# JorgeDFR/nmpc_nav_control

Hardware: AMD Instinct MI355X
Metric: SQP-RTI iterations/sec (whole node), diff N=40 batch=4096; u0 max-abs err (higher is better)
Workload: dtype fp32+fp64; 1 GPU; diff2amr N=40 batch=4096 per GPU; config=metric, N=40, batch_per_gpu=4096, global_batch=4096, parallelism=instance-sharded x1, ranks=1, launcher=single process, closed_loop_warmup_ticks=240, rccl_gather=False, full=False, ipm_rules=product

## Files before the change

### nmpc_nav_control_amd/csrc/sqp_rti_team.hip

```cpp
#include "nmpc_kernels.hpp"
#include "team_common.hpp"
#include "sqp_steps.hpp"
#include "path_march.hpp"

namespace nmpc {

#ifdef NMPC_STAMPS
constexpr int kStampIts = 64;
__device__ unsigned long long g_stamps[256][2 + 4 * kStampIts];
#define STAMP(slot)                                                                                              \
    do {                                                                                                         \
        if (r == 0 && (team & 3) == 0 && (team >> 2) < 256) g_stamps[team >> 2][(slot)] = __builtin_amdgcn_s_memtime(); \
    } while (0)
__device__ unsigned long long g_stamps_p1[256][8];
__device__ unsigned long long g_stamps_pa[256];
__device__ unsigned long long g_stamps_c1[256][kStampIts];
#define STAMPC1()                                                                                                \
    do {                                                                                                         \
        if (it < kStampIts && r == 0 && (team & 3) == 0 && (team >> 2) < 256)                                   \
            g_stamps_c1[team >> 2][it] = __builtin_amdgcn_s_memtime();                                           \
    } while (0)
#define STAMPF(slot)                                                                                             \
    do {                                                                                                         \
        if (it == 2 && k == 20 && r == 0 && (team & 3) == 0 && (team >> 2) < 256)                                 \
            g_stamps_p1[team >> 2][(slot)] = __builtin_amdgcn_s_memtime();                                        \
    } while (0)
#else
#define STAMP(slot) ((void)0)
#define STAMPF(slot) ((void)0)
#define STAMPC1() ((void)0)
#endif

template <class M>
size_t team_scratch_floats(int N, int stride)
{
    return (size_t)stride * (N + 1) * 16 * (TeamRec<M>::RSS + 1) + (size_t)256 * 4 * 16 * (TeamRec<M>::RSS + 1) + 64;
}

namespace {
#ifndef LIGHT_D
#define LIGHT_D 4
#endif
#ifndef LIGHT_DC
#define LIGHT_DC LIGHT_D
#endif
#ifndef P1_D
#define P1_D 2
#endif
#ifdef NMPC_STAMPS
constexpr int kStampItsC = kStampIts;
#else
constexpr int kStampItsC = 0;
#endif

__device__ float g_zero4[4];
__device__ __attribute__((aligned(16))) float g_rec_sentinel[8] = {kFar, kFar, 0.0f, 0.0f, -kFar, kFar, 0.0f, 0.0f};

constexpr int kModeRunPath = 2;
template <class M, bool MS, bool SD, int MODE, bool SP, bool RP, bool MT>
__global__ __launch_bounds__(256, 1) void k_sqp_rti_team(KParams P, KArgs a)
{
    constexpr int mode = MODE == kModeRunPath ? kModeRun : MODE;
    using R = TeamRec<M, SD>;
    constexpr int NX = M::NX, NU = M::NU, NV = R::NV, NGV = R::NGV, RS = R::RS, RSS = R::RSS;
    constexpr bool QM = rec_quad_major<NV>();
    constexpr int KS = 16 * RSS;
    const int gt = blockIdx.x * blockDim.x + threadIdx.x;
    const int team = a.split ? (int)blockIdx.x : (gt >> 4);
    const int row = a.split ? (int)(threadIdx.x >> 4) : 0;
    const int r = gt & 15;
    if (team >= a.B) return;
    if (a.n_active && team >= *a.n_active) return;
    const int N = P.N;
    const size_t S = (size_t)a.stride;
    const size_t Bn = (size_t)a.B;
    const int inst = a.order ? a.order[team] : team;
    const LaneCtx<M> lc = lane_ctx<M, RP>(P, a, inst, r);
    const bool lv = lc.lv, is_u = lc.is_u, is_x = lc.is_x, has_b = lc.has_b;
    const int xi = lc.xi, cx = lc.cx;
    const float sc = P.dt, w_lane = lc.w_lane, h_stage = lc.h_stage, lo_b = lc.lo_b, hi_b = lc.hi_b;
    StageBox sbx{};
    if constexpr (RP) sbx = stage_box_ctx<M, MT>(a, inst, lc, r);
    ModelVals mvals{};
    if constexpr (MT) mvals = robot_vals<M>(P, a, inst);
    const ModelPar mp = MT ? model_par(P, mvals) : model_par(P);
    float* const tbase = a.scratch + (size_t)inst * (N + 1) * KS + (lv ? r : 0) * rec_lane<RSS, QM>();
    float* const tbase_own = a.scratch + (size_t)inst * (N + 1) * KS + r * rec_lane<RSS, QM>();
    float* const tdummy = a.scratch + (size_t)inst * (N + 1) * KS + (size_t)N * KS + 15 * rec_lane<RSS, QM>();
    constexpr bool SPL = R::SPLIT_OK && SP;
    float* const pc0 = a.scratch + (size_t)inst * (N + 1) * KS + (lv ? r : 0) * R::CW;
    float* const pb0 = has_b ? a.scratch + (size_t)inst * (N + 1) * KS + (size_t)(N + 1) * R::CS +
                                   (is_u ? r : NU + (cx >= 0 ? cx : 0)) * R::CW
                             : g_rec_sentinel;
    const int kb = has_b ? R::BS : 0;
    float* const dzbase = a.scratch + (size_t)a.sstride * (N + 1) * KS + (size_t)inst * (N + 1) * 16 + r;
    const bool warm = P.warm && a.warm && a.warm[inst] == a.warm_tag && !(a.reset && a.reset[inst]);

#define XB(k, j) a.xbar[((size_t)(k) * NX + (j)) * S + inst]
#define UBAR(k, j) a.ubar[((size_t)(k) * NU + (j)) * S + inst]

    STAMP(0);
    if (a.reset && a.reset[inst]) {
        for (int k = r; k <= N; k += 16)
            for (int j = 0; j < NX; j++) XB(k, j) = 0.0f;
        for (int k = r; k < N; k += 16)
            for (int j = 0; j < NU; j++) UBAR(k, j) = 0.0f;
        __threadfence_block();
    }

    extern __shared__ double s_path[];
    constexpr bool path = MODE == kModeRunPath;
    const bool traj_lds = path || (a.split && mode == kModeRun);
    const int nslot = a.split ? 1 : 16;
    const int tslot = a.split ? 0 : (int)(threadIdx.x >> 4);
    float* const my_traj = reinterpret_cast<float*>(s_path + nslot * (N + 1)) + (size_t)tslot * (N + 1) * 3;
    float* const s_stg = reinterpret_cast<float*>(s_path) + (traj_lds ? (size_t)nslot * (N + 1) * 5 : 0);
    if (path && row == 0) {
        double* const my_u = s_path + (size_t)tslot * (N + 1);
        const nmpc_path_segment* S = a.segs + (size_t)inst * a.seg_stride;
        const int n = a.nseg[inst];
        if (r == 0) {
            const int cnt = path_march(S, n, a.nearest_u[inst], a.period, N + 1, [&](int j, double su) { my_u[j] = su; });
            for (int j = cnt; j <= N; j++) my_u[j] = (double)n;
        }
        const double* const fr = a.origin();
        const double ox = fr ? fr[inst] : 0.0, oy = fr ? fr[(size_t)a.sstride + inst] : 0.0;
        for (int j = r; j <= N; j += 16) {
            double px, py, pt;
            path_pose(S, n, my_u[j], a.holo, &px, &py, &pt);
            const float fx = (float)(px - ox), fy = (float)(py - oy);
            my_traj[j * 3 + 0] = fx;
            my_traj[j * 3 + 1] = fy;
            my_traj[j * 3 + 2] = (float)pt;
            if (a.traj_out) {
                a.traj_out[((size_t)j * 3 + 0) * Bn + inst] = fx;
                a.traj_out[((size_t)j * 3 + 1) * Bn + inst] = fy;
                a.traj_out[((size_t)j * 3 + 2) * Bn + inst] = (float)pt;
            }
        }
    }

    float x0[NX];
    const X0Lane xl = load_x0<M, RP>(P, a, mode, inst, lc, mp, x0);
    const float pose_th = xl.pose_th, x0_lane = xl.x0_lane;
    float we_lane = xl.we_lane;

    using SL = StageLds<M>;
    if (a.split) {
        const int len_a = (mode == kModeRun) ? ((a.traj_len && !path) ? a.traj_len[inst] : N + 1) : 0;
        struct In {
            float x[NX], u[NU], y, xnext, tq;
            float2 l;
        };
        auto ld = [&](int k, In& v) {
            const int kk = k <= N ? k : N;
#pragma unroll
            for (int j = 0; j < NX; j++) v.x[j] = XB(kk, j);
            const int ku = kk < N ? kk : N - 1;
#pragma unroll
            for (int j = 0; j < NU; j++) v.u[j] = UBAR(ku, j);
            v.xnext = XB(kk < N ? kk + 1 : N, xi);
            v.y = 0.0f;
            v.tq = 0.0f;
            if (mode != kModeRun) {
                const int j = is_u ? NX + r : xi;
                v.y = (lv && j < a.ny_in) ? a.yref[((size_t)kk * a.ny_in + j) * Bn + inst] : 0.0f;
            } else if (!path && r < 3) {
                const int kt = kk < len_a ? kk : (len_a > 0 ? len_a - 1 : 0);
                v.tq = a.traj[((size_t)kt * 3 + r) * Bn + inst];
            }
            v.l = warm ? *reinterpret_cast<const float2*>(SPL ? pb0 + (size_t)kk * kb + 2
                                                              : tbase + (size_t)kk * KS + rec_off<RS, QM>(R::LL))
                       : make_float2(0.0f, 0.0f);
        };
        In cur, nxt;
        ld(row, cur);
        for (int k = row; k <= N; k += 16) {
            ld(k + 16, nxt);
            if (mode == kModeRun && !path && r < 3) my_traj[k * 3 + r] = cur.tq;
            const P0In<M> in = p0_stage_inputs<M>(P, mp, lc, r, k, N, cur.x, cur.u, cur.xnext);
            float* const st = s_stg + SL::at(k, r);
            st[SL::ZBAR] = in.zb;
            st[SL::YREF] = cur.y;
            st[SL::LL] = cur.l.x;
            st[SL::LU] = cur.l.y;
            st[SL::DEFECT] = in.bk;
#pragma unroll
            for (int i = 0; i < NGV; i++) st[SL::gv(i)] = in.g[i];
            cur = nxt;
        }
        __syncthreads();
        if (row != 0) return;
#ifdef NMPC_STAMPS
        if (r == 0 && (team & 3) == 0 && (team >> 2) < 256) g_stamps_pa[team >> 2] = __builtin_amdgcn_s_memtime();
#endif
    }
    const int len = (mode == kModeRun) ? ((a.traj_len && !path) ? a.traj_len[inst] : N + 1) : 0;
    RefUnwrap ref(pose_th);
    float prv_x = 0.0f, prv_y = 0.0f, prv_t = 0.0f;
    auto load_row = [&](int k, float (&xr)[NX], float (&ur)[NU], float (&tr)[3]) {
        const int kk = k <= N ? k : N;
#pragma unroll
        for (int j = 0; j < NX; j++) xr[j] = XB(kk, j);
        const int ku = kk < N ? kk : N - 1;
#pragma unroll
        for (int j = 0; j < NU; j++) ur[j] = UBAR(ku, j);
        if (mode == kModeRun) {
            const int kt = kk < len ? kk : (len > 0 ? len - 1 : 0);
#pragma unroll
            for (int j = 0; j < 3; j++) tr[j] = path ? my_traj[kt * 3 + j] : a.traj[((size_t)kt * 3 + j) * Bn + inst];
        } else {
            tr[0] = tr[1] = tr[2] = 0.0f;
        }
    };
    float xb[NX], ub[NU], tr[3], xb1[NX], ub1[NU], tr1[3];
    load_row(0, xb, ub, tr);
    load_row(1, xb1, ub1, tr1);
    float gcol[NX], grow[NV];
    const_rows<M>(P, mp, lc, r, xb, ub, gcol, grow);
    float dx = is_x ? x0_lane - XB(0, xi) : 0.0f;
    float sum_c0 = 0.0f;
    auto load_l = [&](int k) -> float2 {
        const int kk = k <= N ? k : N;
        const float* const src = warm ? (SPL ? pb0 + (size_t)kk * kb + 2 : tbase + (size_t)kk * KS + rec_off<RS, QM>(R::LL))
                                      : g_zero4;
        return *reinterpret_cast<const float2*>(src);
    };
    auto p0_body = [&](int k, float zbar, float yr_in, const float (&trk)[3], float2 lp, const float (&g)[NX],
                       float bk, float2 box) __attribute__((always_inline)) {
        float yr = yr_in;
        if (mode == kModeRun) {
            ref.step(k < len, trk);
            if (k == N - 1) { prv_x = ref.ref_x; prv_y = ref.ref_y; prv_t = ref.ref_t; }
            float v = 0.0f;
            v = (is_x && xi == 2) ? ref.ref_t : v;
            v = (is_x && xi == 1) ? ref.ref_y : v;
            v = (is_x && xi == 0) ? ref.ref_x : v;
            yr = v;
        }
        float rec[RS];
#pragma unroll
        for (int f = 0; f < RS; f++) rec[f] = 0.0f;
        const bool vu = is_u && k < N, vx = is_x && k >= 1;
        const bool valid = vu || vx;
        float w = sc * w_lane;
        if (k == N) {
            if (mode == kModeRun && P.terminal_hack)
                we_lane = terminal_weight(lc, we_lane, ref.ref_x == prv_x && ref.ref_y == prv_y && ref.ref_t == prv_t);
            w = vx ? we_lane : w;
        }
        rec[R::GR] = valid ? w * (zbar - yr) : 0.0f;
        if constexpr (RP) rec[R::GR] = stage_box_poison(rec[R::GR], box, valid && has_b);
        const float z = vx ? dx : 0.0f;
        rec[R::Z] = z;
        {
            const BoundStart b = bound_start(P, zbar, z, RP ? box.x : lo_b, RP ? box.y : hi_b, warm, lp, valid && has_b);
            rec[R::LB] = b.lb;
            rec[R::UB] = b.ub;
            rec[R::TL] = b.tl;
            rec[R::TU] = b.tu;
            rec[R::LL] = b.ll;
            rec[R::LU] = b.lu;
            sum_c0 += b.c0;
        }
#pragma unroll
        for (int i = 0; i < NGV; i++) rec[R::GV + i] = (k < N && lv) ? g[i] : 0.0f;
        if constexpr (NV > 12) rec_store_range<0, RSS, RS, QM>(tbase_own + (size_t)k * KS, rec);
        else if constexpr (SPL)
            split_store<R, 0, R::GR + 1, RS>(lv ? pc0 + (size_t)k * R::CS : tdummy,
                                             (lv && has_b) ? pb0 + (size_t)k * kb : tdummy + R::CW, rec);
        else rec_store_range<0, RSS, RS, QM>(lv ? tbase + (size_t)k * KS : tdummy, rec);
        dzbase[(size_t)k * 16] = 0.0f;
        if (k < N) {
            const float dzd = is_x ? dx : 0.0f;
            float nxt = dot_v<NX, NU>(0.0f, dzd, grow);
#pragma unroll
            for (int i = 0; i < NGV; i++) {
                const float sr = row_sum16(lv ? g[i] * dzd : 0.0f);
                if (xi == i) nxt = sr;
            }
            dx = is_x ? nxt + bk : 0.0f;
        }
    };
    if (a.split) {
        __builtin_amdgcn_s_waitcnt(0);
        struct Stg {
            float zb, y, ll, lu, b, g[NGV], t[3];
        };
        auto lds_ld = [&](int k, Stg& o) {
            const int kk = k <= N ? k : N;
            const float* const st = s_stg + SL::at(kk, r);
            o.zb = st[SL::ZBAR];
            o.y = st[SL::YREF];
            o.ll = st[SL::LL];
            o.lu = st[SL::LU];
            o.b = st[SL::DEFECT];
#pragma unroll
            for (int i = 0; i < NGV; i++) o.g[i] = st[SL::gv(i)];
#pragma unroll
            for (int j = 0; j < 3; j++) o.t[j] = (mode == kModeRun) ? my_traj[kk * 3 + j] : 0.0f;
        };
        Stg cur, nxt;
        lds_ld(0, cur);
        float2 box = make_float2(lo_b, hi_b), box_n = box;
        if constexpr (RP) box = stage_box<MT>(sbx, 0, N);
        for (int k = 0; k <= N; k++) {
            lds_ld(k + 1, nxt);
            if constexpr (RP) box_n = stage_box<MT>(sbx, k + 1, N);
            float g[NX];
#pragma unroll
            for (int i = 0; i < NX; i++) g[i] = (i < NGV && k < N) ? cur.g[i < NGV ? i : 0] : 0.0f;
            p0_body(k, cur.zb, cur.y, cur.t, make_float2(cur.ll, cur.lu), g, cur.b, box);
            cur = nxt;
            box = box_n;
        }
    } else {
        struct Row {
            float xb[NX], ub[NU], tr[3], yr;
            float2 lp, bx;
        };
        auto load_p0 = [&](int k, Row& o) {
            load_row(k, o.xb, o.ub, o.tr);
            o.lp = load_l(k);
            if constexpr (RP) o.bx = stage_box<MT>(sbx, k, N);
            o.yr = 0.0f;
            if (mode != kModeRun) {
                const int kk = k <= N ? k : N;
                const int j = is_u ? NX + r : xi;
                const bool use = lv && j < a.ny_in;
                const float v = a.yref[((size_t)kk * a.ny_in + (use ? j : 0)) * Bn + inst];
                o.yr = use ? v : 0.0f;
            }
        };
        Row rw[3];
#pragma unroll
        for (int j = 0; j < NX; j++) { rw[0].xb[j] = xb[j]; rw[1].xb[j] = xb1[j]; }
#pragma unroll
        for (int j = 0; j < NU; j++) { rw[0].ub[j] = ub[j]; rw[1].ub[j] = ub1[j]; }
#pragma unroll
        for (int j = 0; j < 3; j++) { rw[0].tr[j] = tr[j]; rw[1].tr[j] = tr1[j]; }
        rw[0].lp = load_l(0);
        rw[1].lp = load_l(1);
        if constexpr (RP) {
            rw[0].bx = stage_box<MT>(sbx, 0, N);
            rw[1].bx = stage_box<MT>(sbx, 1, N);
        }
        rw[0].yr = rw[1].yr = 0.0f;
        if (mode != kModeRun) {
            Row t0, t1;
            load_p0(0, t0);
            load_p0(1, t1);
            rw[0].yr = t0.yr;
            rw[1].yr = t1.yr;
        }
        for (int k0 = 0;; k0 += 3) {
            bool stop = false;
            sfor<0, 3>([&](auto ic) {
                constexpr int i = decltype(ic)::value;
                if (stop) return;
                const int k = k0 + i;
                load_p0(k + 2, rw[(i + 2) % 3]);
                const Row& c = rw[i];
                const Row& n1 = rw[(i + 1) % 3];
                float dxn[NX], g[NX];
#pragma unroll
                for (int q = 0; q < NX; q++) { dxn[q] = 0.0f; g[q] = 0.0f; }
                if (k < N) rk4_column<M>(c.xb, c.ub, P, mp, lv ? r : NU, dxn, g);
                float zbar = 0.0f;
#pragma unroll
                for (int j = 0; j < NU; j++)
                    if (r == j) zbar = c.ub[j];
#pragma unroll
                for (int j = 0; j < NX; j++)
                    if (is_x && xi == j) zbar = c.xb[j];
                float bk = 0.0f;
#pragma unroll
                for (int q = 0; q < NX; q++)
                    if (xi == q) bk = (c.xb[q] - n1.xb[q]) + dxn[q];
                p0_body(k, zbar, c.yr, c.tr, c.lp, g, bk, RP ? c.bx : make_float2(lo_b, hi_b));
                if (k == N) stop = true;
            });
            if (stop) break;
        }
    }
    double onehot[NV];
#pragma unroll
    for (int j = 0; j < NV; j++) onehot[j] = (r == j) ? 1.0 : 0.0;
    double gcol64[NX];
#pragma unroll
    for (int i = 0; i < NX; i++) gcol64[i] = (double)gcol[i];
#ifdef NMPC_MROW
    constexpr bool kMcol = false;
#else
    constexpr bool kMcol = M::kMcolForm;
#endif
    GConst<M> gcs;
    if constexpr (kMcol && !MT) gconst_load<M>(gcs, gcol);

    STAMP(1);
    const float wmax = (RP && a.rparams) ? row_max16(w_lane) : P.wmax;
    const float lam_thr = P.infeas_lam * fmaxf(1.0f, fmaxf(wmax, row_max16(is_x ? we_lane : 0.0f)) * 0.1f);
    const int m = N * NU + N * M::NBX;
    const float inv_m2 = 0.5f / (float)m;
    sum_c0 = row_sum16(lv ? sum_c0 : 0.0f);

    auto p1_load = [&](int kk, float (&v)[RS]) {
        if constexpr (SPL) split_load<R, R::P1L0, R::P1L1, RS>(pc0 + (size_t)kk * R::CS, pb0 + (size_t)kk * kb, v);
        else rec_load_range<R::P1L0, R::P1L1, RS, QM>(tbase + (size_t)kk * KS, v);
        v[R::DZ] = dzbase[(size_t)kk * 16];
    };
    auto sweep = [&](int k0, int k1, int dir, bool ld, auto&& body) {
        const int sd = ld ? dir : 0;
        int kp = k0;
        float ra[RS], rb[RS];
        p1_load(kp, ra);
        for (int k = k0;; k += 2 * dir) {
            const int kp1 = (k == k1) ? kp : kp + sd;
            p1_load(kp1, rb);
            body(k, ra);
            if (k == k1) break;
            const int kp2 = (k + dir == k1) ? kp1 : kp1 + sd;
            p1_load(kp2, ra);
            body(k + dir, rb);
            if (k + dir == k1) break;
            kp = kp2;
        }
    };
    auto sweepd = [&](auto dc, auto f0c, auto fc, int k0, int k1, int dir, bool ld, auto&& body) {
        constexpr int D = decltype(dc)::value;
        constexpr int F0 = decltype(f0c)::value, F = decltype(fc)::value;
        const int sd = ld ? dir : 0;
        float buf[D][RS];
        int kp = k0;
        int kl = k0;
        auto load = [&](int kk, float (&v)[RS]) {
            if constexpr (SPL) split_load<R, F0, F, RS>(pc0 + (size_t)kk * R::CS, pb0 + (size_t)kk * kb, v);
            else rec_load_range<F0, F, RS, QM>(tbase + (size_t)kk * KS, v);
            if constexpr (F == R::P1L1) v[R::DZ] = dzbase[(size_t)kk * 16];
        };
        load(kp, buf[0]);
        sfor<1, D>([&](auto ic) {
            constexpr int i = decltype(ic)::value;
            kp = (kl == k1) ? kp : kp + sd;
            kl = (kl == k1) ? kl : kl + dir;
            load(kp, buf[i]);
        });
        for (int k = k0;; k += D * dir) {
            bool stop = false;
            sfor<0, D>([&](auto ic) {
                constexpr int i = decltype(ic)::value;
                if (stop) return;
                body(k + i * dir, buf[i]);
                if (k + i * dir == k1) {
                    stop = true;
                    return;
                }
                kp = (kl == k1) ? kp : kp + sd;
                kl = (kl == k1) ? kl : kl + dir;
                load(kp, buf[i]);
            });
            if (stop) break;
        }
    };
    int status = 0, it_done = 0;
    bool done = false;
    float exit_res[3] = {0.0f, 0.0f, 0.0f};
    float alpha = 0.0f, sigma_mu = 0.0f, eta = 0.0f, mu_prev = 3.0e38f;
    float tg_rhs = P.sd_hi * sum_c0 * inv_m2;
    for (int it = 0;; it++) {
        double Lrow[NV];
#pragma unroll
        for (int j = 0; j < NV; j++) Lrow[j] = 0.0;
        float pv = 0.0f, piv = 0.0f;
        float res_stat = 0.0f, res_ineq = 0.0f, sum_c = 0.0f, max_c = 0.0f, stat_scale = 1.0f, nanf_ = 0.0f;
        float lam_max = 0.0f;
        bool fail = false;
        const bool act = lv && !done;
        const float a_upd = (it > 0 && !done) ? alpha : 0.0f;
#if P1_D > 2
        sweepd(std::integral_constant<int, P1_D>{}, std::integral_constant<int, R::P1L0>{},
               std::integral_constant<int, R::P1L1>{}, N, 0, -1, act, [&](int k, float (&rc)[RS]) {
#else
        sweep(N, 0, -1, act, [&](int k, float (&rc)[RS]) {
#endif
            STAMPF(0);
            const bool vu = is_u && k < N;
            const bool vx = is_x && k >= 1;
            const bool valid = vu || vx;
            const bool bnd = valid && has_b;
            float z = rc[R::Z];
            float tl = rc[R::TL], tu = rc[R::TU], ll = rc[R::LL], lu = rc[R::LU];
            const float lb = rc[R::LB], ubd = rc[R::UB];
            {
                const float dz = rc[R::DZ];
                const float rl = z - lb - tl, rr = ubd - z - tu;
                const float itl = frcp(tl), itu = frcp(tu);
                float tgl = sigma_mu, tgu = sigma_mu;
                if constexpr (!SD) {
                    const BoundDir da = bound_dir(rc[R::DZA], rl, rr, tl, tu, ll, lu, itl, itu, 0.0f, 0.0f);
                    tgl = sigma_mu - eta * da.dll * da.dtl;
                    tgu = sigma_mu - eta * da.dlu * da.dtu;
                }
                const BoundDir d = bound_dir(dz, rl, rr, tl, tu, ll, lu, itl, itu, tgl, tgu);
                const float ab = bnd ? a_upd : 0.0f, av = valid ? a_upd : 0.0f;
                tl += ab * d.dtl;
                tu += ab * d.dtu;
                ll += ab * d.dll;
                lu += ab * d.dlu;
                z += av * dz;
                rc[R::Z] = z;
                rc[R::TL] = tl;
                rc[R::TU] = tu;
                rc[R::LL] = ll;
                rc[R::LU] = lu;
            }
            const float rl = z - lb - tl, rr = ubd - z - tu;
            const float itl = frcp(tl), itu = frcp(tu);
            res_ineq = fmaxf(res_ineq, fmaxf(fabsf(rl), fabsf(rr)));
            sum_c += ll * tl + lu * tu;
            max_c = fmaxf(max_c, fmaxf(ll * tl, lu * tu));
            lam_max = fmaxf(lam_max, fmaxf(ll, lu));
            const float lamdiff = ll - lu;
            const float sig = ll * itl + lu * itu;
            const float gh = SD ? ll * rl * itl + ll - lu * rr * itu - lu - tg_rhs * itl + tg_rhs * itu
                                : ll * rl * itl + ll - lu * rr * itu - lu;
            STAMPF(1);
            float Gc[NX];
            stage_column<M, R::GV>(rc, gcol, Gc);
            const float cpi = (k < N) ? dot_x<NX, NU>(0.0f, piv, Gc) : 0.0f;
            const float hz = ((k < N) ? h_stage : we_lane) * z;
            const float g = rc[R::GR];
            const float base = hz + g - lamdiff + cpi;
            rc[R::RU] = base;
            res_stat = fmaxf(res_stat, vu ? fabsf(base) : 0.0f);
            stat_scale = fmaxf(stat_scale, vu ? fmaxf(fabsf(cpi), fmaxf(fabsf(g), fabsf(lamdiff))) : 0.0f);
            const float ghat = valid ? (vu ? gh + base : gh) : 0.0f;
            const float pi_new = vx ? base : 0.0f;
            if (ghat != ghat || sig != sig) nanf_ = 1.0f;
            if (k == N) {
                const double d = is_x ? (double)fmaxf(we_lane + sig, 0.0f) : 0.0;
#pragma unroll
                for (int j = 0; j < NV; j++) Lrow[j] = (is_x && j == r) ? d : 0.0;
                pv = is_x ? ghat : 0.0f;
            } else {
                double Gd[NX];
#pragma unroll
                for (int l = 0; l < NX; l++) Gd[l] = (l < NGV) ? (double)Gc[l] : gcol64[l];
                double pg[NX];
#pragma unroll
                for (int i = 0; i < NX; i++) pg[i] = 0.0;
                STAMPF(2);
                pg_block<NX, NU>(pg, Lrow, Gd);
                STAMPF(3);
                const double dg = valid ? (double)h_stage + (double)sig : 1.0;
                double Lr[NV];
#pragma unroll
                for (int j = 0; j < NV; j++) Lr[j] = onehot[j] * dg;
                double pivot;
                bool seq_pivots = true;
                if constexpr (kMcol) {
                    double m11, m10;
                    if constexpr (MT) m_block_team<M>(Lr, pivot, m11, m10, pg, Gd);
                    else m_block<M>(Lr, pivot, m11, m10, pg, Gd, gcs);
                    STAMPF(4);
                    if constexpr (NU == 2 && M::kPivotsUpFront) {
                        chol_input_2<NX>(Lr, pivot, m11, m10, r, fail);
                        seq_pivots = false;
                    } else {
                        (void)m11;
                        (void)m10;
                    }
                } else {
                    mrow_pg_block<NX, NU>(Lr, pivot, pg, Gd);
                    STAMPF(4);
                }
                if (seq_pivots) sfor<0, NU>([&](auto jc) {
                    constexpr int j = decltype(jc)::value;
                    if (!(pivot > 0.0)) fail = true;
                    const double rd = drsq(fmax(pivot, 1e-300));
                    const double lj = (r >= j) ? Lr[j] * rd : 0.0;
                    Lr[j] = lj;
                    chol_update<NX, NU, j>(Lr, lj, pivot);
                });
                STAMPF(5);
                float Lm[NU];
#pragma unroll
                for (int q = 0; q < NU; q++) {
                    Lm[q] = (float)Lr[q];
                    rc[R::LM + q] = Lm[q];
                }
                float y = dot_x<NX, NU>(ghat, pv, Gc);
                float my_lr = 0.0f;
                sfor<0, NU>([&](auto jc) {
                    constexpr int j = decltype(jc)::value;
                    const float lrj = bc<j>(y * frcp(Lm[j]));
                    if (r == j) my_lr = lrj;
                    y -= Lm[j] * lrj;
                });
                rc[R::LR] = my_lr;
                pv = is_x ? y : 0.0f;
#pragma unroll
                for (int j = 0; j < NV; j++) Lrow[j] = Lr[j];
            }
            piv = pi_new;
            STAMPF(6);
            float* const pk = act ? tbase + (size_t)k * KS : tdummy;
            if constexpr (SPL) {
                split_store<R, 0, R::TL, RS>(act ? pc0 + (size_t)k * R::CS : tdummy, tdummy + R::CW, rc);
                split_store<R, R::TL, R::TL + 4, RS>(tdummy, (act && bnd) ? pb0 + (size_t)k * kb : tdummy + R::CW, rc);
            } else if constexpr (MS) {
                rec_store_range<R::TL, R::TL + 4, RS, QM>(bnd ? pk : tdummy, rc);
                if constexpr (R::TL > 0) rec_store_range<0, R::TL, RS, QM>(pk, rc);
                if constexpr (R::TL + 4 < R::P1S1) rec_store_range<R::TL + 4, R::P1S1, RS, QM>(pk, rc);
            } else {
                rec_store_range<0, R::P1S1, RS, QM>(pk, rc);
            }
            STAMPF(7);
        });
        if (it < kStampItsC) STAMP(2 + 4 * it);
        sum_c = row_sum16(lv ? sum_c : 0.0f);
        max_c = row_max16(lv ? max_c : 0.0f);
        lam_max = row_max16(lv ? lam_max : 0.0f);
        res_ineq = row_max16(lv ? res_ineq : 0.0f);
        res_stat = row_max16(lv ? res_stat : 0.0f);
        stat_scale = row_max16(stat_scale);
        nanf_ = row_max16(nanf_);
        const float failf = row_max16(fail ? 1.0f : 0.0f);
        const float mu = sum_c * inv_m2;
        if (!done) {
            exit_res[0] = res_stat;
            exit_res[1] = res_ineq;
            exit_res[2] = mu;
            bool stop = false;
            if (nanf_ > 0.0f || mu != mu) {
                status = 1;
                stop = true;
            } else if (failf > 0.0f) {
                status = (mu <= kBreakdownMuT && res_ineq <= P.tol_ineq * 10.0f) ? 0 : 4;
                stop = true;
            } else if (lam_max > lam_thr && res_ineq > kInfeasRes) {
                status = 4;
                stop = true;
            } else {
                const bool stat_ok = res_stat <= P.tol_stat || res_stat <= kStatRelT * stat_scale;
                const bool cmax_ok = max_c <= kCompMaxRatio * P.tol_comp;
                const bool stalled = mu <= P.tol_comp && mu > 0.5f * mu_prev;
                if (res_ineq <= P.tol_ineq &&
                    ((stat_ok && mu <= P.tol_comp && cmax_ok) || mu <= 1e-2f * P.tol_comp || (stalled && cmax_ok)))
                    stop = true;
                if (it >= P.iter_max) stop = true;
            }
            if (stop) {
                done = true;
                it_done = it;
            }
        }
        mu_prev = mu;
        if (__all(done)) break;

        float sigma = 0.0f, alpha_aff = 0.0f;
        for (int pass = SD ? 1 : 0; pass < (SD ? 2 : 3); pass++) {
            bool run = !done;
            if (SD) {
                sigma_mu = tg_rhs;
                eta = 0.0f;
            } else if (pass == 1) {
                sigma_mu = sigma * mu;
                eta = alpha_aff;
            } else if (pass == 2) {
                if (__all(done || alpha >= 0.1f)) break;
                run = run && alpha < 0.1f;
                sigma_mu = run ? fmaxf(sigma, 0.3f) * mu : sigma_mu;
                eta = run ? 0.0f : eta;
            }
            const bool ld = lv && run;
            if (!SD && pass > 0) {
                float pvc = 0.0f;
                sweepd(std::integral_constant<int, LIGHT_DC>{}, std::integral_constant<int, 0>{}, std::integral_constant<int, R::NB>{}, N, 0, -1, ld, [&](int k, float (&rc)[RS]) {
                    const bool vu = is_u && k < N;
                    float ghat;
                    {
                        const float z = rc[R::Z];
                        const float tl = rc[R::TL], tu = rc[R::TU], ll = rc[R::LL], lu = rc[R::LU];
                        const float rl = z - rc[R::LB] - tl, rr = rc[R::UB] - z - tu;
                        const float itl = frcp(tl), itu = frcp(tu);
                        const BoundDir da = bound_dir(rc[R::DZA], rl, rr, tl, tu, ll, lu, itl, itu, 0.0f, 0.0f);
                        const float tgl = sigma_mu - eta * da.dll * da.dtl, tgu = sigma_mu - eta * da.dlu * da.dtu;
                        ghat = -(tgl - ll * rl) * itl + ll + (tgu - lu * rr) * itu - lu;
                    }
                    ghat += vu ? rc[R::RU] : 0.0f;
                    if (k == N) {
                        pvc = is_x ? ghat : 0.0f;
                    } else {
                        float Gc[NX];
                        stage_column<M, R::GV>(rc, gcol, Gc);
                        float y = dot_x<NX, NU>(ghat, pvc, Gc);
                        float my_lr = 0.0f;
                        sfor<0, NU>([&](auto jc) {
                            constexpr int j = decltype(jc)::value;
                            const float Lmj = rc[R::LM + j];
                            const float lrj = bc<j>(y * frcp(Lmj));
                            if (r == j) my_lr = lrj;
                            y -= Lmj * lrj;
                        });
                        if (ld && is_u) (SPL ? pc0[(size_t)k * R::CS] : tbase[(size_t)k * KS + rec_off<RS, QM>(R::LR)]) = my_lr;
                        rc[R::LR] = my_lr;
                        pvc = is_x ? y : 0.0f;
                    }
                });
            }
            if (pass == 1) STAMPC1();
            float amax = 1e30f, s1 = 0.0f, s2 = 0.0f;
            auto fwd = [&](auto cc) {
            constexpr int kind = decltype(cc)::value;
            constexpr bool corr = kind != 0;
            float dxs = 0.0f;
            sweepd(std::integral_constant<int, LIGHT_D>{}, std::integral_constant<int, 0>{}, std::integral_constant<int, R::NF>{}, 0, N, 1, ld, [&](int k, float (&rc)[RS]) {
                const bool vu = is_u && k < N;
                const bool vx = is_x && k >= 1;
                const bool valid = vu || vx;
                float du_all[NU];
#pragma unroll
                for (int q = 0; q < NU; q++) du_all[q] = 0.0f;
                if (NU == 2 || k < N) {
                    float w[NU];
                    sfor<0, NU>([&](auto qc) {
                        constexpr int q = decltype(qc)::value;
                        w[q] = bc<q>(rc[R::LR]) + ((k > 0) ? row_sum16(is_x ? rc[R::LM + q] * dxs : 0.0f) : 0.0f);
                    });
                    sfor<0, NU>([&](auto qqc) {
                        constexpr int q = NU - 1 - decltype(qqc)::value;
                        float sq = w[q];
                        sfor<q + 1, NU>([&](auto jc) {
                            constexpr int j = decltype(jc)::value;
                            sq -= bc<j>(rc[R::LM + q]) * du_all[j];
                        });
                        du_all[q] = sq * frcp(bc<q>(rc[R::LM + q]));
                    });
#pragma unroll
                    for (int q = 0; q < NU; q++) du_all[q] = (k < N) ? -du_all[q] : 0.0f;
                }
                float dz = 0.0f;
#pragma unroll
                for (int q = 0; q < NU; q++)
                    if (r == q) dz = du_all[q];
                dz = is_x ? ((k >= 1) ? dxs : 0.0f) : dz;
                {
                    const float z = rc[R::Z];
                    const float tl = rc[R::TL], tu = rc[R::TU], ll = rc[R::LL], lu = rc[R::LU];
                    const float rl = z - rc[R::LB] - tl, rr = rc[R::UB] - z - tu;
                    const float itl = frcp(tl), itu = frcp(tu);
                    float tgl = 0.0f, tgu = 0.0f;
                    if (kind == 1) {
                        const BoundDir da = bound_dir(rc[R::DZA], rl, rr, tl, tu, ll, lu, itl, itu, 0.0f, 0.0f);
                        tgl = sigma_mu - eta * da.dll * da.dtl;
                        tgu = sigma_mu - eta * da.dlu * da.dtu;
                    } else if (kind == 2) {
                        tgl = sigma_mu;
                        tgu = sigma_mu;
                    }
                    const BoundDir d = bound_dir(dz, rl, rr, tl, tu, ll, lu, itl, itu, tgl, tgu);
                    amax = step_bound_r(amax, tl, d.dtl);
                    amax = step_bound_r(amax, tu, d.dtu);
                    amax = step_bound_r(amax, ll, d.dll);
                    amax = step_bound_r(amax, lu, d.dlu);
                    if (kind == 0) {
                        s1 += ll * d.dtl + tl * d.dll + lu * d.dtu + tu * d.dlu;
                        s2 += d.dll * d.dtl + d.dlu * d.dtu;
                    } else if (kind == 2) {
                        const bool bnd = valid && has_b;
                        s1 += bnd ? ll * d.dtl + tl * d.dll + lu * d.dtu + tu * d.dlu : 0.0f;
                        s2 += bnd ? d.dll * d.dtl + d.dlu * d.dtu : 0.0f;
                    }
                }
                {
                    const bool st = ld && valid;
                    if (corr) *(st ? dzbase + (size_t)k * 16 : tdummy) = dz;
                    else
                        *((st && !SPL) ? tbase + (size_t)k * KS + rec_off<RS, QM>(R::DZA) : tdummy) = dz;
                }
                if (k < N) dxs = stage_dyn<M, R::GV>(lc, rc, valid ? dz : 0.0f, grow);
            });
            };
            if constexpr (SD) fwd(std::integral_constant<int, 2>{});
            else if (pass == 0) fwd(std::integral_constant<int, 0>{});
            else fwd(std::integral_constant<int, 1>{});
            amax = row_min16(lv ? amax : 1e30f);
            if (SD) {
                s1 = row_sum16(lv ? s1 : 0.0f);
                s2 = row_sum16(lv ? s2 : 0.0f);
                if (run) alpha = fminf(1.0f, P.tau * amax);
                const float mu_next = fmaxf((sum_c + alpha * s1 + alpha * alpha * s2) * inv_m2, 0.0f);
                const float om = 1.0f - alpha;
                tg_rhs = fminf(fmaxf(om * om, P.sd_lo), P.sd_hi) * mu_next;
                if (it < kStampItsC) STAMP(4 + 4 * it);
            } else if (pass == 0) {
                s1 = row_sum16(lv ? s1 : 0.0f);
                s2 = row_sum16(lv ? s2 : 0.0f);
                alpha_aff = fminf(1.0f, amax);
                const float mu_aff = (sum_c + alpha_aff * s1 + alpha_aff * alpha_aff * s2) * inv_m2;
                float sg = (mu > 0.0f) ? mu_aff / mu : 0.0f;
                sg = fmaxf(sg, 0.0f);
                sigma = fminf(sg * sg * sg, 1.0f);
                if (it < kStampItsC) STAMP(3 + 4 * it);
            } else {
                if (run) alpha = fminf(1.0f, P.tau * amax);
                if (pass == 1 && it < kStampItsC) STAMP(4 + 4 * it);
            }
        }
        if (it < kStampItsC) STAMP(5 + 4 * it);
    }

    if (status == 0) {
        auto entry = [&](int k) -> float* {
            const int kk = k <= N ? k : N;
            float* const px = &XB(kk, xi);
            float* const pu = &UBAR(kk < N ? kk : N - 1, is_u ? r : 0);
            return is_x ? px : ((is_u && kk < N) ? pu : tdummy);
        };
        sqp_full_step(N, is_x, x0_lane, entry, [&](int kk) {
            return SPL ? pc0[(size_t)kk * R::CS + R::Z] : tbase[(size_t)kk * KS + rec_off<RS, QM>(R::Z)];
        });
        if (a.xtraj || a.utraj) {
            __threadfence_block();
            for (int k = 0; k <= N; k++) {
                if (is_x && a.xtraj) a.xtraj[((size_t)k * NX + xi) * Bn + inst] = XB(k, xi);
                if (is_u && k < N && a.utraj) a.utraj[((size_t)k * NU + r) * Bn + inst] = UBAR(k, r);
            }
        }
    }
    __threadfence_block();
    if (r == 0) write_outputs<M>(P, a, mp, mode, inst, status, it_done, exit_res, x0);
#undef XB
#undef UBAR
}

}

template <class M>
hipError_t launch_sqp_rti_team(const KParams& P, const KArgs& a, int mode, hipStream_t stream)
{
    if (a.B <= 0) return hipSuccess;
    const size_t stg = (size_t)(P.N + 1) * 16 * StageLds<M>::SF * sizeof(float);
    const size_t split_lds = stg + (mode == kModeRun ? (sizeof(double) + 3 * sizeof(float)) * (size_t)(P.N + 1) : 0);
    KArgs as = a;
    if (as.split && split_lds > 65536) as.split = 0;
    const int block = 256;
    const long long threads = (long long)a.B * (as.split ? 256 : 16);
    const int grid = (int)((threads + block - 1) / block);
    const size_t lds = as.split ? split_lds
                                : ((mode == kModeRun && a.segs) ? (sizeof(double) + 3 * sizeof(float)) * 16 * (size_t)(P.N + 1) : 0);
    if (lds > 65536) return hipErrorInvalidValue;
    auto go = [&](auto kern) { hipLaunchKernelGGL(kern, dim3(grid), dim3(block), lds, stream, P, as); };
    const int km = mode != kModeRun ? kModeSolve : (a.segs ? kModeRunPath : kModeRun);
    auto pick2 = [&](auto msc, auto sdc, auto spc) {
        constexpr bool ms = decltype(msc)::value, sd = decltype(sdc)::value, sp = decltype(spc)::value;
        auto pick3 = [&](auto rpc, auto mtc) {
            constexpr bool rp = decltype(rpc)::value, mt = decltype(mtc)::value;
            if (km == kModeRunPath) go(k_sqp_rti_team<M, ms, sd, kModeRunPath, sp, rp, mt>);
            else if (km == kModeRun) go(k_sqp_rti_team<M, ms, sd, kModeRun, sp, rp, mt>);
            else go(k_sqp_rti_team<M, ms, sd, kModeSolve, sp, rp, mt>);
        };
        if (a.rmodel) pick3(std::true_type{}, std::true_type{});
        else if (a.rparams || a.sbounds) pick3(std::true_type{}, std::false_type{});
        else pick3(std::false_type{}, std::false_type{});
    };
    auto pick = [&](auto msc, auto sdc) {
        using R = TeamRec<M, decltype(sdc)::value>;
        if constexpr (R::SPLIT) pick2(msc, sdc, std::true_type{});
        else if constexpr (R::SPLIT_OK) {
            if (a.rec_split) pick2(msc, sdc, std::true_type{});
            else pick2(msc, sdc, std::false_type{});
        } else pick2(msc, sdc, std::false_type{});
    };
    using T = std::true_type;
    using F = std::false_type;
    if (P.ipm == 1) {
        if (a.dense) pick(T{}, T{});
        else pick(F{}, T{});
    } else if (a.dense) {
        pick(T{}, F{});
    } else {
        pick(F{}, F{});
    }
    return hipGetLastError();
}

template hipError_t launch_sqp_rti_team<Diff2>(const KParams&, const KArgs&, int, hipStream_t);
template hipError_t launch_sqp_rti_team<Omni4>(const KParams&, const KArgs&, int, hipStream_t);
template hipError_t launch_sqp_rti_team<Tric3>(const KParams&, const KArgs&, int, hipStream_t);
template size_t team_scratch_floats<Diff2>(int, int);
template size_t team_scratch_floats<Omni4>(int, int);
template size_t team_scratch_floats<Tric3>(int, int);

#ifdef NMPC_STAMPS
extern "C" int nmpc_debug_stamps_c1(unsigned long long* host)
{
    return hipMemcpyFromSymbol(host, HIP_SYMBOL(g_stamps_c1), sizeof(g_stamps_c1), 0, hipMemcpyDeviceToHost) == hipSuccess ? 0 : -2;
}
extern "C" int nmpc_debug_stamps_pa(unsigned long long* host)
{
    return hipMemcpyFromSymbol(host, HIP_SYMBOL(g_stamps_pa), sizeof(g_stamps_pa), 0, hipMemcpyDeviceToHost) == hipSuccess ? 0 : -2;
}
extern "C" int nmpc_debug_stamps_p1(unsigned long long* host)
{
    return hipMemcpyFromSymbol(host, HIP_SYMBOL(g_stamps_p1), sizeof(g_stamps_p1), 0, hipMemcpyDeviceToHost) == hipSuccess ? 0 : -2;
}
extern "C" int nmpc_debug_stamps(unsigned long long* host, int n)
{
    const size_t bytes = sizeof(unsigned long long) * (size_t)n;
    if (bytes > sizeof(g_stamps)) return -1;
    return hipMemcpyFromSymbol(host, HIP_SYMBOL(g_stamps), bytes, 0, hipMemcpyDeviceToHost) == hipSuccess ? 0 : -2;
}
#endif

}
```

Baseline: 4.363 million SQP-RTI iterations/sec.

## Peel first and tail stages of Riccati sweeps to drop per-stage boundary checks

Restructures the record-prefetching sweep into a peeled first stage, a steady-state loop with no boundary tests (stage kind known at compile time), and a peeled tail. Boundary predicates like k==N or k<N become compile-time constants in the mid loop, with sched_barriers placed between stages. It also rewrites some multiply-add pairs into explicit fma form. This removes per-stage index clamping and branching in the hot backward and forward sweeps, at the cost of more code size and instruction-cache pressure, and the fma regrouping slightly changes float rounding.

```diff
diff --git a/nmpc_nav_control_amd/csrc/sqp_rti_team.hip b/nmpc_nav_control_amd/csrc/sqp_rti_team.hip
--- a/nmpc_nav_control_amd/csrc/sqp_rti_team.hip
+++ b/nmpc_nav_control_amd/csrc/sqp_rti_team.hip
@@ -2,6 +2,7 @@
 #include "team_common.hpp"
 #include "sqp_steps.hpp"
 #include "path_march.hpp"
+#include "sweep_plan.hpp"
 
 namespace nmpc {
 
@@ -52,6 +53,42 @@
 #else
 constexpr int kStampItsC = 0;
 #endif
+
+constexpr int kStAny = 0, kStFirst = 1, kStMid = 2, kStRest = 3, kStBoth = 4;
+template <int EK, bool BACK>
+__device__ __forceinline__ bool at_top(int k, int N)
+{
+    if constexpr (EK == kStMid) return false;
+    else if constexpr (EK == kStFirst) return BACK;
+    else if constexpr (EK == kStRest && BACK) return false;
+    else return k == N;
+}
+template <int EK, bool BACK>
+__device__ __forceinline__ bool at_zero(int k)
+{
+    if constexpr (EK == kStMid) return false;
+    else if constexpr (EK == kStFirst) return !BACK;
+    else if constexpr (EK == kStRest && !BACK) return false;
+    else return k == 0;
+}
+template <int EK, bool BACK>
+__device__ __forceinline__ bool below_top(int k, int N)
+{
+    if constexpr (EK == kStAny) return k < N;
+    else return !at_top<EK, BACK>(k, N);
+}
+template <int EK, bool BACK>
+__device__ __forceinline__ bool past_zero(int k)
+{
+    if constexpr (EK == kStAny) return k >= 1;
+    else return !at_zero<EK, BACK>(k);
+}
+__device__ __forceinline__ float fma_ab_cd(float a, float b, float c, float d) { return __builtin_fmaf(a, b, c * d); }
+#define NMPC_STR_(x) #x
+#define NMPC_STR(x) NMPC_STR_(x)
+constexpr bool kSweepGeneric = sizeof(NMPC_STR(NMPC_SWEEP_GENERIC)) != sizeof("NMPC_SWEEP_GENERIC");
+#undef NMPC_STR
+#undef NMPC_STR_
 
 __device__ float g_zero4[4];
 __device__ __attribute__((aligned(16))) float g_rec_sentinel[8] = {kFar, kFar, 0.0f, 0.0f, -kFar, kFar, 0.0f, 0.0f};
@@ -404,64 +441,109 @@
     const float inv_m2 = 0.5f / (float)m;
     sum_c0 = row_sum16(lv ? sum_c0 : 0.0f);
 
-    auto p1_load = [&](int kk, float (&v)[RS]) {
-        if constexpr (SPL) split_load<R, R::P1L0, R::P1L1, RS>(pc0 + (size_t)kk * R::CS, pb0 + (size_t)kk * kb, v);
-        else rec_load_range<R::P1L0, R::P1L1, RS, QM>(tbase + (size_t)kk * KS, v);
-        v[R::DZ] = dzbase[(size_t)kk * 16];
-    };
-    auto sweep = [&](int k0, int k1, int dir, bool ld, auto&& body) {
-        const int sd = ld ? dir : 0;
-        int kp = k0;
-        float ra[RS], rb[RS];
-        p1_load(kp, ra);
-        for (int k = k0;; k += 2 * dir) {
-            const int kp1 = (k == k1) ? kp : kp + sd;
-            p1_load(kp1, rb);
-            body(k, ra);
-            if (k == k1) break;
-            const int kp2 = (k + dir == k1) ? kp1 : kp1 + sd;
-            p1_load(kp2, ra);
-            body(k + dir, rb);
-            if (k + dir == k1) break;
-            kp = kp2;
-        }
-    };
-    auto sweepd = [&](auto dc, auto f0c, auto fc, int k0, int k1, int dir, bool ld, auto&& body) {
+    auto sweepd = [&](auto dc, auto f0c, auto fc, auto backc, bool ld, auto&& body) {
         constexpr int D = decltype(dc)::value;
         constexpr int F0 = decltype(f0c)::value, F = decltype(fc)::value;
+        constexpr bool BACK = decltype(backc)::value;
+        constexpr int dir = BACK ? -1 : 1;
+        static_assert(D >= 2, "at least two record buffers");
+        const int k0 = BACK ? N : 0, k1 = BACK ? 0 : N;
         const int sd = ld ? dir : 0;
         float buf[D][RS];
-        int kp = k0;
-        int kl = k0;
         auto load = [&](int kk, float (&v)[RS]) {
             if constexpr (SPL) split_load<R, F0, F, RS>(pc0 + (size_t)kk * R::CS, pb0 + (size_t)kk * kb, v);
             else rec_load_range<F0, F, RS, QM>(tbase + (size_t)kk * KS, v);
             if constexpr (F == R::P1L1) v[R::DZ] = dzbase[(size_t)kk * 16];
         };
-        load(kp, buf[0]);
-        sfor<1, D>([&](auto ic) {
-            constexpr int i = decltype(ic)::value;
-            kp = (kl == k1) ? kp : kp + sd;
-            kl = (kl == k1) ? kl : kl + dir;
-            load(kp, buf[i]);
-        });
-        for (int k = k0;; k += D * dir) {
+        if constexpr (kSweepGeneric) {
+            constexpr std::integral_constant<int, kStAny> any{};
+            if constexpr (D == 2) {
+                int kp = k0;
+                load(kp, buf[0]);
+                for (int k = k0;; k += 2 * dir) {
+                    const int kp1 = (k == k1) ? kp : kp + sd;
+                    load(kp1, buf[1]);
+                    body(any, k, buf[0]);
+                    if (k == k1) break;
+                    const int kp2 = (k + dir == k1) ? kp1 : kp1 + sd;
+                    load(kp2, buf[0]);
+                    body(any, k + dir, buf[1]);
+                    if (k + dir == k1) break;
+                    kp = kp2;
+                }
+                return;
+            }
+            int kp = k0;
+            int kl = k0;
+            load(kp, buf[0]);
+            sfor<1, D>([&](auto ic) {
+                constexpr int i = decltype(ic)::value;
+                kp = (kl == k1) ? kp : kp + sd;
+                kl = (kl == k1) ? kl : kl + dir;
+                load(kp, buf[i]);
+            });
+            for (int k = k0;; k += D * dir) {
+                bool stop = false;
+                sfor<0, D>([&](auto ic) {
+                    constexpr int i = decltype(ic)::value;
+                    if (stop) return;
+                    body(std::integral_constant<int, kStAny>{}, k + i * dir, buf[i]);
+                    if (k + i * dir == k1) {
+                        stop = true;
+                        return;
+                    }
+                    kp = (kl == k1) ? kp : kp + sd;
+                    kl = (kl == k1) ? kl : kl + dir;
+                    load(kp, buf[i]);
+                });
+                if (stop) break;
+            }
+        } else {
+            int kp = k0;
+            load(kp, buf[0]);
+            sfor<1, D>([&](auto ic) {
+                constexpr int i = decltype(ic)::value;
+                kp += (i <= N) ? sd : 0;
+                load(kp, buf[i]);
+            });
+            body(std::integral_constant<int, kStFirst>{}, k0, buf[0]);
+            kp += (D <= N) ? sd : 0;
+            load(kp, buf[0]);
+            int k = k0 + dir;
+            const int T = sweep_full_trips(N, D);
+            asm volatile("; sweep: first stage done");
+            for (int t = 0; t < T; t++) {
+                sfor<0, D>([&](auto ic) {
+                    constexpr int i = decltype(ic)::value;
+                    constexpr int b = (i + 1) % D;
+                    __builtin_amdgcn_sched_barrier(0);
+                    body(std::integral_constant<int, kStMid>{}, k + i * dir, buf[b]);
+                    kp += sd;
+                    load(kp, buf[b]);
+                });
+                k += D * dir;
+            }
+            int jl = sweep_loaded_before_rest(N, D);
             bool stop = false;
-            sfor<0, D>([&](auto ic) {
+            sfor<0, sweep_rest_max(D)>([&](auto ic) {
                 constexpr int i = decltype(ic)::value;
+                constexpr int b = (i + 1) % D;
                 if (stop) return;
-                body(k + i * dir, buf[i]);
+                body(std::integral_constant<int, kStRest>{}, k + i * dir, buf[b]);
                 if (k + i * dir == k1) {
                     stop = true;
                     return;
                 }
-                kp = (kl == k1) ? kp : kp + sd;
-                kl = (kl == k1) ? kl : kl + dir;
-                load(kp, buf[i]);
+                if constexpr (sweep_rest_refills(i, D)) {
+                    kp = (jl == N) ? kp : kp + sd;
+                    jl = (jl == N) ? jl : jl + 1;
+                    load(kp, buf[b]);
+                }
             });
-            if (stop) break;
         }
     };
+    constexpr std::integral_constant<bool, true> kBackward{};
+    constexpr std::integral_constant<bool, false> kForward{};
     int status = 0, it_done = 0;
     bool done = false;
     float exit_res[3] = {0.0f, 0.0f, 0.0f};
@@ -477,15 +559,14 @@
         bool fail = false;
         const bool act = lv && !done;
         const float a_upd = (it > 0 && !done) ? alpha : 0.0f;
-#if P1_D > 2
         sweepd(std::integral_constant<int, P1_D>{}, std::integral_constant<int, R::P1L0>{},
-               std::integral_constant<int, R::P1L1>{}, N, 0, -1, act, [&](int k, float (&rc)[RS]) {
-#else
-        sweep(N, 0, -1, act, [&](int k, float (&rc)[RS]) {
-#endif
+               std::integral_constant<int, R::P1L1>{}, kBackward, act, [&](auto ekc, int k, float (&rc)[RS]) {
+            constexpr int ekv = decltype(ekc)::value;
+            constexpr int ek = ekv == kStRest ? kStBoth : ekv;
+            const bool kN = at_top<ek, true>(k, N), ltN = below_top<ek, true>(k, N);
             STAMPF(0);
-            const bool vu = is_u && k < N;
-            const bool vx = is_x && k >= 1;
+            const bool vu = is_u && ltN;
+            const bool vx = is_x && past_zero<ek, true>(k);
             const bool valid = vu || vx;
             const bool bnd = valid && has_b;
             float z = rc[R::Z];
@@ -517,18 +598,18 @@
             const float rl = z - lb - tl, rr = ubd - z - tu;
             const float itl = frcp(tl), itu = frcp(tu);
             res_ineq = fmaxf(res_ineq, fmaxf(fabsf(rl), fabsf(rr)));
-            sum_c += ll * tl + lu * tu;
+            sum_c += fma_ab_cd(ll, tl, lu, tu);
             max_c = fmaxf(max_c, fmaxf(ll * tl, lu * tu));
             lam_max = fmaxf(lam_max, fmaxf(ll, lu));
             const float lamdiff = ll - lu;
-            const float sig = ll * itl + lu * itu;
+            const float sig = fma_ab_cd(ll, itl, lu, itu);
             const float gh = SD ? ll * rl * itl + ll - lu * rr * itu - lu - tg_rhs * itl + tg_rhs * itu
                                 : ll * rl * itl + ll - lu * rr * itu - lu;
             STAMPF(1);
             float Gc[NX];
             stage_column<M, R::GV>(rc, gcol, Gc);
-            const float cpi = (k < N) ? dot_x<NX, NU>(0.0f, piv, Gc) : 0.0f;
-            const float hz = ((k < N) ? h_stage : we_lane) * z;
+            const float cpi = ltN ? dot_x<NX, NU>(0.0f, piv, Gc) : 0.0f;
+            const float hz = (ltN ? h_stage : we_lane) * z;
             const float g = rc[R::GR];
             const float base = hz + g - lamdiff + cpi;
             rc[R::RU] = base;
@@ -537,7 +618,7 @@
             const float ghat = valid ? (vu ? gh + base : gh) : 0.0f;
             const float pi_new = vx ? base : 0.0f;
             if (ghat != ghat || sig != sig) nanf_ = 1.0f;
-            if (k == N) {
+            if (kN) {
                 const double d = is_x ? (double)fmaxf(we_lane + sig, 0.0f) : 0.0;
 #pragma unroll
                 for (int j = 0; j < NV; j++) Lrow[j] = (is_x && j == r) ? d : 0.0;
@@ -676,8 +757,9 @@
             const bool ld = lv && run;
             if (!SD && pass > 0) {
                 float pvc = 0.0f;
-                sweepd(std::integral_constant<int, LIGHT_DC>{}, std::integral_constant<int, 0>{}, std::integral_constant<int, R::NB>{}, N, 0, -1, ld, [&](int k, float (&rc)[RS]) {
-                    const bool vu = is_u && k < N;
+                sweepd(std::integral_constant<int, LIGHT_DC>{}, std::integral_constant<int, 0>{}, std::integral_constant<int, R::NB>{}, kBackward, ld, [&](auto ekc, int k, float (&rc)[RS]) {
+                    const bool kN = at_top<decltype(ekc)::value, true>(k, N);
+                    const bool vu = is_u && below_top<decltype(ekc)::value, true>(k, N);
                     float ghat;
                     {
                         const float z = rc[R::Z];
@@ -689,7 +771,7 @@
                         ghat = -(tgl - ll * rl) * itl + ll + (tgu - lu * rr) * itu - lu;
                     }
                     ghat += vu ? rc[R::RU] : 0.0f;
-                    if (k == N) {
+                    if (kN) {
                         pvc = is_x ? ghat : 0.0f;
                     } else {
                         float Gc[NX];
@@ -715,18 +797,20 @@
             constexpr int kind = decltype(cc)::value;
             constexpr bool corr = kind != 0;
             float dxs = 0.0f;
-            sweepd(std::integral_constant<int, LIGHT_D>{}, std::integral_constant<int, 0>{}, std::integral_constant<int, R::NF>{}, 0, N, 1, ld, [&](int k, float (&rc)[RS]) {
-                const bool vu = is_u && k < N;
-                const bool vx = is_x && k >= 1;
+            sweepd(std::integral_constant<int, LIGHT_D>{}, std::integral_constant<int, 0>{}, std::integral_constant<int, R::NF>{}, kForward, ld, [&](auto ekc, int k, float (&rc)[RS]) {
+                constexpr int ek = decltype(ekc)::value;
+                const bool ltN = below_top<ek, false>(k, N), gt0 = past_zero<ek, false>(k);
+                const bool vu = is_u && ltN;
+                const bool vx = is_x && gt0;
                 const bool valid = vu || vx;
                 float du_all[NU];
 #pragma unroll
                 for (int q = 0; q < NU; q++) du_all[q] = 0.0f;
-                if (NU == 2 || k < N) {
+                if (NU == 2 || ltN) {
                     float w[NU];
                     sfor<0, NU>([&](auto qc) {
                         constexpr int q = decltype(qc)::value;
-                        w[q] = bc<q>(rc[R::LR]) + ((k > 0) ? row_sum16(is_x ? rc[R::LM + q] * dxs : 0.0f) : 0.0f);
+                        w[q] = bc<q>(rc[R::LR]) + (gt0 ? row_sum16(is_x ? rc[R::LM + q] * dxs : 0.0f) : 0.0f);
                     });
                     sfor<0, NU>([&](auto qqc) {
                         constexpr int q = NU - 1 - decltype(qqc)::value;
@@ -738,13 +822,13 @@
                         du_all[q] = sq * frcp(bc<q>(rc[R::LM + q]));
                     });
 #pragma unroll
-                    for (int q = 0; q < NU; q++) du_all[q] = (k < N) ? -du_all[q] : 0.0f;
+                    for (int q = 0; q < NU; q++) du_all[q] = ltN ? -du_all[q] : 0.0f;
                 }
                 float dz = 0.0f;
 #pragma unroll
                 for (int q = 0; q < NU; q++)
                     if (r == q) dz = du_all[q];
-                dz = is_x ? ((k >= 1) ? dxs : 0.0f) : dz;
+                dz = is_x ? (gt0 ? dxs : 0.0f) : dz;
                 {
                     const float z = rc[R::Z];
                     const float tl = rc[R::TL], tu = rc[R::TU], ll = rc[R::LL], lu = rc[R::LU];
@@ -765,12 +849,12 @@
                     amax = step_bound_r(amax, ll, d.dll);
                     amax = step_bound_r(amax, lu, d.dlu);
                     if (kind == 0) {
-                        s1 += ll * d.dtl + tl * d.dll + lu * d.dtu + tu * d.dlu;
-                        s2 += d.dll * d.dtl + d.dlu * d.dtu;
+                        s1 += fma_ab_cd(ll, d.dtl, tl, d.dll) + lu * d.dtu + tu * d.dlu;
+                        s2 += fma_ab_cd(d.dll, d.dtl, d.dlu, d.dtu);
                     } else if (kind == 2) {
                         const bool bnd = valid && has_b;
-                        s1 += bnd ? ll * d.dtl + tl * d.dll + lu * d.dtu + tu * d.dlu : 0.0f;
-                        s2 += bnd ? d.dll * d.dtl + d.dlu * d.dtu : 0.0f;
+                        s1 += bnd ? fma_ab_cd(ll, d.dtl, tl, d.dll) + lu * d.dtu + tu * d.dlu : 0.0f;
+                        s2 += bnd ? fma_ab_cd(d.dll, d.dtl, d.dlu, d.dtu) : 0.0f;
                     }
                 }
                 {
@@ -779,7 +863,7 @@
                     else
                         *((st && !SPL) ? tbase + (size_t)k * KS + rec_off<RS, QM>(R::DZA) : tdummy) = dz;
                 }
-                if (k < N) dxs = stage_dyn<M, R::GV>(lc, rc, valid ? dz : 0.0f, grow);
+                if (ltN) dxs = stage_dyn<M, R::GV>(lc, rc, valid ? dz : 0.0f, grow);
             });
             };
             if constexpr (SD) fwd(std::integral_constant<int, 2>{});
diff --git a/nmpc_nav_control_amd/csrc/sweep_plan.hpp b/nmpc_nav_control_amd/csrc/sweep_plan.hpp
--- /dev/null
+++ b/nmpc_nav_control_amd/csrc/sweep_plan.hpp
@@ -0,0 +1,14 @@
+#pragma once
+
+namespace nmpc {
+
+constexpr int sweep_full_trips(int N, int D) { return N / D - 1 > 0 ? N / D - 1 : 0; }
+constexpr int sweep_loaded_before_rest(int N, int D)
+{
+    return (sweep_full_trips(N, D) + 1) * D < N ? (sweep_full_trips(N, D) + 1) * D : N;
+}
+constexpr int sweep_rest_stages(int N, int D) { return N - sweep_full_trips(N, D) * D; }
+constexpr bool sweep_rest_refills(int i, int D) { return i <= D - 2; }
+constexpr int sweep_rest_max(int D) { return 2 * D - 1; }
+
+}
```

Measured after the change: 4.433 million SQP-RTI iterations/sec, median of 6. 1.6% higher.
